# ShangtongZhang/DistributedES

Measured on NVIDIA H100. Metric: nes_policy_evals_per_sec, higher is better.
Workload: dtype f16x3 (split-fp16 operands ~ f32, f32 accumulate)

## Files before the change

### distributedes_b200/csrc/des_eval_tc.cu

```cuda
#include "des_common.cuh"
#include "des_tc.cuh"

namespace des {

using namespace tc;

constexpr int kK1 = 32;
constexpr int kMaxA = 8;
constexpr int kProdWGs = 2;
constexpr int kProdThreads = 128 * kProdWGs;
constexpr int kTcThreads = kProdThreads + 256;
constexpr int kConsWarps = 8;
template <int H, bool X3, int NA>
__host__ __device__ constexpr uint32_t prod_regs() { return (H == 256 && X3 && NA == 8) ? 40u : 56u; }
template <int H, bool X3, int NA>
__host__ __device__ constexpr uint32_t cons_regs() { return (((65536u / kTcThreads) & ~7u) * kTcThreads - kProdThreads * prod_regs<H, X3, NA>()) / 256u & ~7u; }
static_assert(cons_regs<256, true, 4>() == 200 && cons_regs<256, true, 8>() == 216, "register split");

#ifdef DES_EVAL_TRACE
enum { TR_WAIT, TR_MMA, TR_SYNC, TR_EPI, TR_GEN, TR_OTHER, TR_N };
#define DES_TRACE_INIT uint32_t tr_[TR_N] = {}; long long tr_t = clock64(), tr_0 = tr_t;
#define DES_TRACE(k) do { const long long t_ = clock64(); tr_[k] += (uint32_t)(t_ - tr_t); tr_t = t_; } while (0)
#define DES_TRACE_PRINT(role, members)                                                                                \
    if (blockIdx.x < 2 && lane == 0)                                                                                  \
        printf("DES_TRACE cta=%d warp=%d role=%s members=%d wait=%u mma=%u sync=%u epi=%u gen=%u other=%u total=%u\n", \
               (int)blockIdx.x, warp, role, members, tr_[TR_WAIT], tr_[TR_MMA], tr_[TR_SYNC], tr_[TR_EPI], tr_[TR_GEN],  \
               tr_[TR_OTHER], (uint32_t)(clock64() - tr_0))
#else
#define DES_TRACE_INIT
#define DES_TRACE(k)
#define DES_TRACE_PRINT(role, members)
#endif

template <int H, bool X3>
struct TcCfg {
    static constexpr int NCH = H / 64;
    static constexpr int KAT = H / 64;
    static constexpr int KS2 = H / 16;
    static constexpr int PLANES = X3 ? 2 : 1;
    static constexpr int CHUNK_BYTES = PLANES * KAT * 8192;
    static constexpr int W1_BYTES = PLANES * H * 128;
    static constexpr int SMALL_FLOATS = 2 * H + kMaxA * H + kMaxA;
    enum { BAR_W2_FULL = 0, BAR_W2_EMPTY = 2, BAR_W1_FULL = 4, BAR_W1_EMPTY = 5, BAR_SMALL_EMPTY = 6, NBARS = 8 };
    static constexpr size_t OFF_W1 = 2 * (size_t)CHUNK_BYTES;
    static constexpr size_t OFF_SMALL = OFF_W1 + W1_BYTES;
    static constexpr size_t OFF_FIT = OFF_SMALL + 2 * (size_t)SMALL_FLOATS * sizeof(float);
    static constexpr size_t OFF_CNT = OFF_FIT + 2 * kConsWarps * sizeof(float);
    static constexpr size_t OFF_BAR = (OFF_CNT + 2 * sizeof(uint32_t) + 7) & ~(size_t)7;
    static constexpr size_t SMEM = 1024 + OFF_BAR + NBARS * sizeof(uint64_t);
    static_assert(SMEM <= 227 * 1024, "eval_tc_kernel: shared memory over the 227 KB per-block limit");
    static_assert(SMALL_FLOATS * sizeof(float) % 16 == 0, "small-array buffers must stay float4 aligned");
};

struct TcArgs {
    float *fitness;
    const float *theta, *obs, *target;
    const des_state *state;
    Layout L;
    int T, n_pass;
    float sigma, clip, neg2ln2_sigma2;
    PhiloxKey key;
    uint32_t gen;
    uint64_t member_offset;
    int64_t n_local;
    uint8_t *cache;
};

__device__ __forceinline__ float perturbed1(const float *__restrict__ theta, int j, float sigma, uint32_t member,
                                            uint32_t gen, const PhiloxKey &key) {
    const float4 z = noise_quad((uint32_t)(j >> 2), member, gen, kStreamNesEps, key);
    const int e = j & 3;
    const float zz = e == 0 ? z.x : (e == 1 ? z.y : (e == 2 ? z.z : z.w));
    return __fmaf_rn(sigma, zz, __ldg(theta + j));
}

template <bool kMirror>
__device__ __forceinline__ float4 member_quad(uint32_t q, uint32_t member, uint32_t gen, const PhiloxKey &key,
                                              float neg2ln2_sigma2, float4 base, float sgn) {
    if (!kMirror) return perturbed_quad(q, member, gen, kStreamNesEps, key, neg2ln2_sigma2, base);
    const uint4 x = philox4x32(q, member, gen, kStreamNesEps, key);
    const BmParts a = box_muller_parts(x.x, x.y, neg2ln2_sigma2, key.one_bits);
    const BmParts b = box_muller_parts(x.z, x.w, neg2ln2_sigma2, key.one_bits);
    const float ra = a.nr * sgn, rb = b.nr * sgn;
    return make_float4(__fmaf_rn(ra, a.c, base.x), __fmaf_rn(ra, a.s, base.y), __fmaf_rn(rb, b.c, base.z),
                       __fmaf_rn(rb, b.s, base.w));
}

template <bool X3>
__device__ __forceinline__ void octet(const float (&w)[8], uint4 &hi, uint4 &lo) {
    if (X3) {
        split_h2(w[0], w[1], hi.x, lo.x); split_h2(w[2], w[3], hi.y, lo.y);
        split_h2(w[4], w[5], hi.z, lo.z); split_h2(w[6], w[7], hi.w, lo.w);
    } else {
        hi = make_uint4(pack_h2(w[0], w[1]), pack_h2(w[2], w[3]), pack_h2(w[4], w[5]), pack_h2(w[6], w[7]));
        lo = hi;
    }
}

template <bool X3>
__device__ __forceinline__ void load_x(uint32_t (&xh)[2][4], uint32_t (&xl)[2][4], const float *__restrict__ obs, int d0,
                                       int ra, int lane) {
#pragma unroll
    for (int ks = 0; ks < 2; ++ks) {
#pragma unroll
        for (int i = 0; i < 4; ++i) {
            const int row = ra + (i & 1) * 8, k = ks * 16 + (i >> 1) * 8 + (lane & 3) * 2;
            const float v0 = k < d0 ? __ldg(obs + (int64_t)row * d0 + k) : 0.f;
            const float v1 = k + 1 < d0 ? __ldg(obs + (int64_t)row * d0 + k + 1) : 0.f;
            if (X3) split_h2(v0, v1, xh[ks][i], xl[ks][i]);
            else xh[ks][i] = pack_h2(v0, v1);
        }
    }
}

template <int H, bool X3, int CL, int NA, bool kMirror>
__device__ __forceinline__ void eval_tc_body(const TcArgs &a) {
    using C = TcCfg<H, X3>;
    extern __shared__ __align__(1024) uint8_t smem_raw[];
    uint8_t *smem = reinterpret_cast<uint8_t *>((reinterpret_cast<uintptr_t>(smem_raw) + 1023) & ~(uintptr_t)1023);
    uint8_t *w2buf = smem;
    uint8_t *w1 = smem + C::OFF_W1;
    float *small_buf = reinterpret_cast<float *>(smem + C::OFF_SMALL);
    float *fit_part = reinterpret_cast<float *>(smem + C::OFF_FIT);
    uint32_t *fit_cnt = reinterpret_cast<uint32_t *>(smem + C::OFF_CNT);
    const uint32_t bars = smem_u32(smem + C::OFF_BAR);
    auto bar = [&](int k) { return bars + 8u * (uint32_t)k; };

    const int tid = threadIdx.x, warp = tid >> 5, lane = tid & 31;
    const uint32_t rank = CL == 2 ? cluster_ctarank() : 0u;
    const Layout L = a.L;
    const uint32_t gen = generation_word(a.state, a.gen);
    const int64_t first = blockIdx.x / CL, stride = gridDim.x / CL;

    constexpr uint32_t kW2Copy = (64 / CL) * 128, kW2Copies = C::PLANES * C::KAT;
    constexpr uint32_t kW1Copy = (H / CL) * 128, kW1Copies = C::PLANES;
    static_assert(CL * kW2Copies * kW2Copy == C::CHUNK_BYTES && CL * kW1Copies * kW1Copy == C::W1_BYTES,
                  "the two halves must make up the whole tile, or a full barrier never completes");
    static_assert(kW2Copy % 16 == 0 && kW1Copy % 16 == 0, "bulk copies move multiples of 16 bytes");
    static_assert(kW2Copies * kW2Copy < (1u << 20) && kW1Copies * kW1Copy < (1u << 20), "mbarrier tx-count range");

    if (tid == 0) {
        for (int s = 0; s < 2; ++s) {
            mbar_init(bar(C::BAR_W2_FULL + s), 1);
            mbar_init(bar(C::BAR_W2_EMPTY + s), kConsWarps * CL);
            mbar_init(bar(C::BAR_SMALL_EMPTY + s), kTcThreads - kProdThreads);
        }
        mbar_init(bar(C::BAR_W1_FULL), 1);
        mbar_init(bar(C::BAR_W1_EMPTY), kConsWarps * CL);
        fit_cnt[0] = fit_cnt[1] = 0u;
        fence_barrier_init();
    }
    if (CL == 2) cluster_sync_relaxed();
    __syncthreads();
    const uint32_t peer_bars = CL == 2 ? map_cluster(bars, rank ^ 1u) : 0u;
    auto release_all = [&](int k) {
        mbar_arrive(bar(k));
        if (CL == 2) mbar_arrive_remote(peer_bars + 8u * (uint32_t)k);
    };

    if (warp < 4 * kProdWGs) {
        setmaxnreg_dec<prod_regs<H, X3, NA>()>();
        DES_TRACE_INIT
        const int ptid = tid;
        uint8_t *const cache = (a.cache && a.n_pass > 1) ? a.cache + (size_t)blockIdx.x * C::NCH * C::CHUNK_BYTES : nullptr;
        auto put = [&](uint8_t *base, uint32_t off, uint32_t lo_off, const uint4 &hi, const uint4 &lo) {
            *reinterpret_cast<uint4 *>(base + off) = hi;
            if (X3) *reinterpret_cast<uint4 *>(base + lo_off + off) = lo;
        };
        auto publish = [&](int k, uint32_t base, uint32_t bytes, uint32_t ncopy, uint32_t step) {
            fence_proxy_async_cta();
            named_bar_sync(1, kProdThreads);
            if (ptid == 0) {
                if (CL == 2) {
                    mbar_expect_tx(bar(k), ncopy * bytes);
                    const uint32_t peer_bar = map_cluster(bar(k), rank ^ 1u);
                    for (uint32_t j = 0; j < ncopy; ++j) {
                        const uint32_t src = base + j * step + rank * bytes;
                        bulk_copy_to_peer(map_cluster(src, rank ^ 1u), src, bytes, peer_bar);
                    }
                } else {
                    mbar_arrive(bar(k));
                }
            }
        };
        constexpr int kOct = H / 8;
        constexpr int kRows = 64 / CL;
        auto gen_chunk = [&](uint32_t member, float sgn, int c, int pass, int buf) {
            uint8_t *dst = w2buf + buf * C::CHUNK_BYTES;
            uint8_t *mirror = cache ? cache + (size_t)c * C::CHUNK_BYTES : nullptr;
            for (int idx = ptid; idx < kRows * kOct; idx += kProdThreads) {
                const int rr = (int)rank * kRows + idx / kOct, o = idx % kOct;
                const uint32_t off = (uint32_t)((o >> 3) * 8192 + rr * 128 + (((o & 7) ^ (rr & 7)) << 4));
                uint4 hi, lo;
                if (mirror && pass > 0) {
                    hi = *reinterpret_cast<const uint4 *>(mirror + off);
                    if (X3) lo = *reinterpret_cast<const uint4 *>(mirror + C::KAT * 8192 + off);
                    else lo = hi;
                } else {
                    const int j0 = L.off_w2 + (c * 64 + rr) * H + o * 8;
                    const float4 p0 = member_quad<kMirror>((uint32_t)(j0 >> 2), member, gen, a.key, a.neg2ln2_sigma2,
                                                           __ldg(reinterpret_cast<const float4 *>(a.theta + j0)), sgn);
                    const float4 p1 = member_quad<kMirror>((uint32_t)(j0 >> 2) + 1, member, gen, a.key, a.neg2ln2_sigma2,
                                                           __ldg(reinterpret_cast<const float4 *>(a.theta + j0 + 4)), sgn);
                    const float w[8] = {p0.x, p0.y, p0.z, p0.w, p1.x, p1.y, p1.z, p1.w};
                    octet<X3>(w, hi, lo);
                    if (mirror) {
                        *reinterpret_cast<uint4 *>(mirror + off) = hi;
                        if (X3) *reinterpret_cast<uint4 *>(mirror + C::KAT * 8192 + off) = lo;
                    }
                }
                put(dst, off, C::KAT * 8192, hi, lo);
            }
        };

        uint32_t q = 0;
        int i = 0;
        for (int64_t m = first; m < a.n_local; m += stride, ++i) {
            const uint32_t member = noise_word(a.member_offset + (uint64_t)m, kMirror);
            const float sgn = member_sigma(a.member_offset + (uint64_t)m, kMirror, 1.0f);
            float *small = small_buf + (i & 1) * C::SMALL_FLOATS;
            if (i >= 2) mbar_wait(bar(C::BAR_SMALL_EMPTY + (i & 1)), ((i >> 1) - 1) & 1);
            DES_TRACE(TR_WAIT);
            for (int k = ptid; k < H / 4; k += kProdThreads) {
                const float4 v1 = member_quad<kMirror>((uint32_t)((L.off_b1 >> 2) + k), member, gen, a.key, a.neg2ln2_sigma2,
                                                       __ldg(reinterpret_cast<const float4 *>(a.theta + L.off_b1) + k), sgn);
                const float4 v2 = member_quad<kMirror>((uint32_t)((L.off_b2 >> 2) + k), member, gen, a.key, a.neg2ln2_sigma2,
                                                       __ldg(reinterpret_cast<const float4 *>(a.theta + L.off_b2) + k), sgn);
                const float bsc = X3 ? kTwoLog2e : 1.0f;
                reinterpret_cast<float4 *>(small)[k] = make_float4(v1.x * bsc, v1.y * bsc, v1.z * bsc, v1.w * bsc);
                reinterpret_cast<float4 *>(small + H)[k] = make_float4(v2.x * bsc, v2.y * bsc, v2.z * bsc, v2.w * bsc);
            }
            for (int k = ptid; k < L.A * H / 4; k += kProdThreads)
                reinterpret_cast<float4 *>(small + 2 * H)[k] =
                    member_quad<kMirror>((uint32_t)((L.off_w3 >> 2) + k), member, gen, a.key, a.neg2ln2_sigma2,
                                         __ldg(reinterpret_cast<const float4 *>(a.theta + L.off_w3) + k), sgn);
            for (int k = L.A * H + ptid; k < H * kMaxA; k += kProdThreads) small[2 * H + k] = 0.f;
            if (ptid < kMaxA)
                small[2 * H + kMaxA * H + ptid] = ptid < L.A ? perturbed1(a.theta, L.off_b3 + ptid, sgn * a.sigma, member, gen, a.key) : 0.f;
            DES_TRACE(TR_GEN);
            if (i >= 1) mbar_wait(bar(C::BAR_W1_EMPTY), (i - 1) & 1);
            DES_TRACE(TR_WAIT);
            for (int idx = ptid; idx < (H / CL) * 4; idx += kProdThreads) {
                const int n = (int)rank * (H / CL) + (idx >> 2), c8 = idx & 3;
                float w[8];
                if ((L.d0 & 3) == 0) {
#pragma unroll
                    for (int hq = 0; hq < 2; ++hq) {
                        const int k = c8 * 8 + hq * 4;
                        float4 v = make_float4(0.f, 0.f, 0.f, 0.f);
                        if (k < L.d0) {
                            const int j = L.off_w1 + n * L.d0 + k;
                            v = member_quad<kMirror>((uint32_t)(j >> 2), member, gen, a.key, a.neg2ln2_sigma2,
                                                     __ldg(reinterpret_cast<const float4 *>(a.theta + j)), sgn);
                        }
                        w[4 * hq] = v.x; w[4 * hq + 1] = v.y; w[4 * hq + 2] = v.z; w[4 * hq + 3] = v.w;
                    }
                } else {
#pragma unroll
                    for (int e = 0; e < 8; ++e) {
                        const int k = c8 * 8 + e;
                        w[e] = (k < L.d0) ? perturbed1(a.theta, L.off_w1 + n * L.d0 + k, sgn * a.sigma, member, gen, a.key) : 0.f;
                    }
                }
                uint4 hi, lo;
                octet<X3>(w, hi, lo);
                put(w1, (uint32_t)(n * 128 + ((c8 ^ (n & 7)) << 4)), H * 128, hi, lo);
            }
            DES_TRACE(TR_GEN);
            publish(C::BAR_W1_FULL, smem_u32(w1), kW1Copy, kW1Copies, H * 128);
            DES_TRACE(TR_SYNC);
            for (int pass = 0; pass < a.n_pass; ++pass) {
                for (int c = 0; c < C::NCH; ++c, ++q) {
                    const int s = (int)(q & 1u);
                    if (q >= 2) mbar_wait(bar(C::BAR_W2_EMPTY + s), ((q >> 1) - 1) & 1u);
                    DES_TRACE(TR_WAIT);
                    gen_chunk(member, sgn, c, pass, s);
                    DES_TRACE(TR_GEN);
                    publish(C::BAR_W2_FULL + s, smem_u32(w2buf + s * C::CHUNK_BYTES), kW2Copy, kW2Copies, 8192);
                    DES_TRACE(TR_SYNC);
                }
            }
        }
        if (CL == 2) {
            for (uint32_t t = q > 2u ? q - 2u : 0u; t < q; ++t) mbar_wait(bar(C::BAR_W2_EMPTY + (int)(t & 1u)), (t >> 1) & 1u);
            if (i >= 1) mbar_wait(bar(C::BAR_W1_EMPTY), (i - 1) & 1);
        }
        DES_TRACE_PRINT("producer", i);
    } else {
        setmaxnreg_inc<cons_regs<H, X3, NA>()>();
        DES_TRACE_INIT
        const int cwarp = warp - 4 * kProdWGs, cw = cwarp >> 2;
        const int r_in_tile = cw * 64 + (cwarp & 3) * 16 + (lane >> 2);
        const int cq = (lane & 3) * 2;
        uint32_t q = 0;
        int i = 0;
        for (int64_t m = first; m < a.n_local; m += stride, ++i) {
            const float *small = small_buf + (i & 1) * C::SMALL_FLOATS;
            const float *b1 = small, *b2 = small + H, *w3 = small + 2 * H, *b3 = small + 2 * H + kMaxA * H;
            mbar_wait(bar(C::BAR_W1_FULL), (uint32_t)i & 1u);
            DES_TRACE(TR_WAIT);

            float sq = 0.f;
            for (int pass = 0; pass < a.n_pass; ++pass) {
                const int tile = pass * CL + (int)rank;
                const int ra = tile * 128 + r_in_tile;
                uint32_t h1h[C::KS2][4], h1l[X3 ? C::KS2 : 1][4];
                {
                    uint32_t xh[2][4], xl[2][4];
                    load_x<X3>(xh, xl, a.obs, L.d0, ra, lane);
                    DES_TRACE(TR_OTHER);
#pragma unroll
                    for (int c = 0; c < C::NCH; ++c) {
                        float d[32];
#pragma unroll
                        for (int k = 0; k < 32; ++k) d[k] = 0.f;
                        wgmma_fence();
#pragma unroll
                        for (int ks = 0; ks < 2; ++ks) {
                            const uint32_t bh = smem_u32(w1) + c * 8192 + ks * 32;
                            wgmma_rs_n64(d, xh[ks], smem_desc_sw128(bh), ks > 0);
                            if (X3) {
                                wgmma_rs_n64(d, xl[ks], smem_desc_sw128(bh), 1);
                                wgmma_rs_n64(d, xh[ks], smem_desc_sw128(bh + H * 128), 1);
                            }
                        }
                        wgmma_commit();
                        wgmma_wait<0>();
                        fence_regs(d);
                        DES_TRACE(TR_MMA);
                        if (c == C::NCH - 1 && pass == a.n_pass - 1 && lane == 0) release_all(C::BAR_W1_EMPTY);
                        DES_TRACE(TR_SYNC);
#pragma unroll
                        for (int j = 0; j < 8; ++j) {
                            const float2 b = *reinterpret_cast<const float2 *>(b1 + c * 64 + j * 8 + cq);
                            const int s = c * 4 + (j >> 1), e = (j & 1) * 2;
#pragma unroll
                            for (int r = 0; r < 2; ++r) {
                                const float v0 = d[4 * j + 2 * r], v1 = d[4 * j + 2 * r + 1];
                                if (X3) split_h2(tanh_acc_b(v0, b.x), tanh_acc_b(v1, b.y), h1h[s][e + r], h1l[s][e + r]);
                                else h1h[s][e + r] = pack_h2(tanh_fast(v0 + b.x), tanh_fast(v1 + b.y));
                            }
                        }
                        DES_TRACE(TR_EPI);
                    }
                }
                float act[NA][2];
#pragma unroll
                for (int k = 0; k < NA; ++k) act[k][0] = act[k][1] = 0.f;
                for (int c = 0; c < C::NCH; ++c, ++q) {
                    const int st = (int)(q & 1u);
                    mbar_wait(bar(C::BAR_W2_FULL + st), (q >> 1) & 1u);
                    DES_TRACE(TR_WAIT);
                    const uint32_t bbase = smem_u32(w2buf + st * C::CHUNK_BYTES);
                    float d[32];
#pragma unroll
                    for (int k = 0; k < 32; ++k) d[k] = 0.f;
                    wgmma_fence();
#pragma unroll
                    for (int s = 0; s < C::KS2; ++s) {
                        const uint32_t bh = bbase + (s >> 2) * 8192 + (s & 3) * 32;
                        wgmma_rs_n64(d, h1h[s], smem_desc_sw128(bh), s > 0);
                        if (X3) {
                            wgmma_rs_n64(d, h1l[s], smem_desc_sw128(bh), 1);
                            wgmma_rs_n64(d, h1h[s], smem_desc_sw128(bh + C::KAT * 8192), 1);
                        }
                    }
                    wgmma_commit();
                    wgmma_wait<0>();
                    fence_regs(d);
                    DES_TRACE(TR_MMA);
                    if (lane == 0) release_all(C::BAR_W2_EMPTY + st);
                    DES_TRACE(TR_SYNC);
#pragma unroll
                    for (int j = 0; j < 8; ++j) {
                        const int n = c * 64 + j * 8 + cq;
                        const float2 b = *reinterpret_cast<const float2 *>(b2 + n);
#pragma unroll
                        for (int r = 0; r < 2; ++r) {
                            float h0, h1;
                            if (X3) {
                                h0 = tanh_acc_b(d[4 * j + 2 * r], b.x);
                                h1 = tanh_acc_b(d[4 * j + 2 * r + 1], b.y);
                            } else {
                                h0 = tanh_fast(d[4 * j + 2 * r] + b.x);
                                h1 = tanh_fast(d[4 * j + 2 * r + 1] + b.y);
                            }
#pragma unroll
                            for (int k = 0; k < NA; ++k) {
                                if (k < L.A) {
                                    const float2 w = *reinterpret_cast<const float2 *>(w3 + k * H + n);
                                    act[k][r] = __fmaf_rn(h1, w.y, __fmaf_rn(h0, w.x, act[k][r]));
                                }
                            }
                        }
                    }
                    DES_TRACE(TR_EPI);
                }
#pragma unroll
                for (int k = 0; k < NA; ++k) {
#pragma unroll
                    for (int r = 0; r < 2; ++r) {
                        act[k][r] += __shfl_xor_sync(0xffffffffu, act[k][r], 1);
                        act[k][r] += __shfl_xor_sync(0xffffffffu, act[k][r], 2);
                    }
                }
                if ((lane & 3) == 0) {
#pragma unroll
                    for (int r = 0; r < 2; ++r) {
                        const int t = ra + 8 * r;
#pragma unroll
                        for (int k = 0; k < NA; ++k) {
                            if (k < L.A) {
                                float v = act[k][r] + b3[k];
                                v = clip_keep_nan(v, a.clip);
                                const float dd = v - __ldg(a.target + (int64_t)t * L.A + k);
                                sq = __fmaf_rn(dd, dd, sq);
                            }
                        }
                    }
                }
            }
#pragma unroll
            for (int o = 16; o > 0; o >>= 1) sq += __shfl_xor_sync(0xffffffffu, sq, o);
            if (lane == 0) {
                float *part = fit_part + (i & 1) * kConsWarps;
                part[cwarp] = sq;
                __threadfence_block();
                if (atomicAdd(fit_cnt + (i & 1), 1u) == kConsWarps - 1) {
                    __threadfence_block();
                    double f = 0.0;
                    for (int w = 0; w < kConsWarps; ++w) f += (double)reinterpret_cast<volatile float *>(part)[w];
                    fit_cnt[i & 1] = 0u;
                    if (CL == 2) atomicAdd(a.fitness + m, (float)(-f));
                    else a.fitness[m] = (float)(-f);
                }
            }
            mbar_arrive(bar(C::BAR_SMALL_EMPTY + (i & 1)));
            DES_TRACE(TR_OTHER);
        }
        DES_TRACE_PRINT("consumer", i);
    }
}

template <int H, bool X3, int CL, int NA>
__global__ void __launch_bounds__(kTcThreads, 1) eval_tc_kernel(TcArgs a) { eval_tc_body<H, X3, CL, NA, false>(a); }

template <int H, bool X3, int CL, int NA>
__global__ void __launch_bounds__(kTcThreads, 1) eval_tc_mirrored_kernel(TcArgs a) { eval_tc_body<H, X3, CL, NA, true>(a); }

template <int H, bool X3, int CL, int NA, bool kMirror>
static int launch_tc(TcArgs &a, cudaStream_t st) {
    using C = TcCfg<H, X3>;
    const auto kernel = kMirror ? eval_tc_mirrored_kernel<H, X3, CL, NA> : eval_tc_kernel<H, X3, CL, NA>;
    a.n_pass = a.T / 128 / CL;
    int dev = 0, sms = 132;
    DES_CUDA(cudaGetDevice(&dev));
    DES_CUDA(cudaDeviceGetAttribute(&sms, cudaDevAttrMultiProcessorCount, dev));
    if (CL == 2) {
        DES_CUDA(cudaFuncSetAttribute(kernel, cudaFuncAttributeMaxDynamicSharedMemorySize, (int)C::SMEM));
        DES_CUDA(cudaMemsetAsync(a.fitness, 0, (size_t)a.n_local * sizeof(float), st));
        const int64_t clusters = a.n_local < sms / 2 ? a.n_local : sms / 2;
        cudaLaunchConfig_t cfg = {};
        cfg.gridDim = dim3((unsigned)(2 * clusters));
        cfg.blockDim = dim3(kTcThreads);
        cfg.dynamicSmemBytes = C::SMEM;
        cfg.stream = st;
        cudaLaunchAttribute attr[1];
        attr[0].id = cudaLaunchAttributeClusterDimension;
        attr[0].val.clusterDim.x = 2;
        attr[0].val.clusterDim.y = 1;
        attr[0].val.clusterDim.z = 1;
        cfg.attrs = attr;
        cfg.numAttrs = 1;
        DES_CUDA(cudaLaunchKernelEx(&cfg, kernel, a));
        DES_LAUNCH_CHECK("eval_tc_kernel");
        return DES_OK;
    }
    const int64_t grid = a.n_local < sms ? a.n_local : sms;
    return launch_smem("eval_tc_kernel", kernel, (unsigned)grid, kTcThreads, C::SMEM, st, a);
}

template <int H, bool X3, bool kMirror>
static int launch_tc_m(TcArgs &a, cudaStream_t st) {
    const bool even = (a.T / 128) % 2 == 0;
    if (a.L.A <= 4) return even ? launch_tc<H, X3, 2, 4, kMirror>(a, st) : launch_tc<H, X3, 1, 4, kMirror>(a, st);
    return even ? launch_tc<H, X3, 2, kMaxA, kMirror>(a, st) : launch_tc<H, X3, 1, kMaxA, kMirror>(a, st);
}

template <int H, bool X3>
static int launch_tc_h(TcArgs &a, bool mirrored, cudaStream_t st) {
    return mirrored ? launch_tc_m<H, X3, true>(a, st) : launch_tc_m<H, X3, false>(a, st);
}

static int tc_passes(int T) { const int tiles = T / 128; return tiles % 2 == 0 ? tiles / 2 : tiles; }

size_t eval_tc_workspace_bytes(des_dims dims, int precision) {
    const int H = dims.hidden;
    if (!(H == 64 || H == 128 || H == 256) || dims.tape_len % 128 != 0 || tc_passes(dims.tape_len) <= 1) return 0;
    int dev = 0, sms = 132;
    if (cudaGetDevice(&dev) != cudaSuccess || cudaDeviceGetAttribute(&sms, cudaDevAttrMultiProcessorCount, dev) != cudaSuccess) {
        cudaGetLastError();
        sms = 132;
    }
    return (size_t)sms * (size_t)H * H * 2 * (precision == DES_FWD_F16X3 ? 2 : 1);
}

int eval_tc_launch(float *fitness, const float *theta, const float *obs, const float *target, des_dims dims,
                   double sigma, double clip, uint64_t seed, uint64_t generation, const des_state *state,
                   int64_t member_offset, int64_t n_local, int precision, void *workspace, size_t workspace_bytes,
                   bool mirrored, cudaStream_t st) {
    const int H = dims.hidden;
    if (!(H == 64 || H == 128 || H == 256) || dims.state_dim > kK1 || dims.action_dim > kMaxA || dims.tape_len % 128 != 0) {
        set_error("des_nes_eval(tensor): needs hidden in {64,128,256}, state_dim <= %d, action_dim <= %d, tape_len %% 128 == 0 "
                  "(got d0=%d H=%d A=%d T=%d); use DES_FWD_FP32 for other shapes", kK1, kMaxA, dims.state_dim, H,
                  dims.action_dim, dims.tape_len);
        return DES_ERR_UNSUPPORTED;
    }
    if (((uintptr_t)theta & 15) != 0) {
        set_error("des_nes_eval(tensor): theta_dev must be 16-byte aligned");
        return DES_ERR_INVALID_ARGUMENT;
    }
    TcArgs a;
    a.fitness = fitness; a.theta = theta; a.obs = obs; a.target = target; a.state = state;
    a.L = Layout(dims.state_dim, H, dims.action_dim);
    a.T = dims.tape_len;
    a.sigma = (float)sigma; a.clip = (float)clip;
    a.neg2ln2_sigma2 = kNeg2Ln2 * (float)sigma * (float)sigma;
    a.key = make_philox_key(seed); a.gen = (uint32_t)generation;
    a.member_offset = (uint64_t)member_offset; a.n_local = n_local;
    const bool x3 = precision == DES_FWD_F16X3;
    const size_t need = eval_tc_workspace_bytes(dims, precision);
    a.cache = (need > 0 && workspace && workspace_bytes >= need && ((uintptr_t)workspace & 15) == 0) ? (uint8_t *)workspace : nullptr;
    switch (H) {
        case 64: return x3 ? launch_tc_h<64, true>(a, mirrored, st) : launch_tc_h<64, false>(a, mirrored, st);
        case 128: return x3 ? launch_tc_h<128, true>(a, mirrored, st) : launch_tc_h<128, false>(a, mirrored, st);
        default: return x3 ? launch_tc_h<256, true>(a, mirrored, st) : launch_tc_h<256, false>(a, mirrored, st);
    }
}

}
```

### distributedes_b200/csrc/des_tc.cuh

```cuda
#pragma once
#include <cuda_fp16.h>
#include <stdint.h>

namespace des {
namespace tc {

__device__ __forceinline__ uint32_t smem_u32(const void *p) { return (uint32_t)__cvta_generic_to_shared(p); }

__device__ __forceinline__ void mbar_init(uint32_t bar, uint32_t count) {
    asm volatile("mbarrier.init.shared::cta.b64 [%0], %1;" ::"r"(bar), "r"(count) : "memory");
}
__device__ __forceinline__ void fence_barrier_init() { asm volatile("fence.mbarrier_init.release.cluster;" ::: "memory"); }
__device__ __forceinline__ bool mbar_try_wait(uint32_t bar, uint32_t parity) {
    uint32_t ok;
    asm volatile(
        "{\n\t.reg .pred p;\n\t"
        "mbarrier.try_wait.parity.shared::cta.b64 p, [%1], %2, %3;\n\t"
        "selp.u32 %0, 1, 0, p;\n\t}"
        : "=r"(ok) : "r"(bar), "r"(parity), "r"(1000000u) : "memory");
    return ok != 0;
}
__device__ __forceinline__ void mbar_wait(uint32_t bar, uint32_t parity) {
    while (!mbar_try_wait(bar, parity)) {
    }
}
__device__ __forceinline__ void mbar_arrive(uint32_t bar) {
    asm volatile("mbarrier.arrive.shared::cta.b64 _, [%0];" ::"r"(bar) : "memory");
}
__device__ __forceinline__ void mbar_arrive_remote(uint32_t cbar) {
    asm volatile("mbarrier.arrive.shared::cluster.b64 _, [%0];" ::"r"(cbar) : "memory");
}
__device__ __forceinline__ void mbar_expect_tx(uint32_t bar, uint32_t bytes) {
    asm volatile("mbarrier.arrive.expect_tx.shared::cta.b64 _, [%0], %1;" ::"r"(bar), "r"(bytes) : "memory");
}
__device__ __forceinline__ void fence_proxy_async_cta() { asm volatile("fence.proxy.async.shared::cta;" ::: "memory"); }
__device__ __forceinline__ void named_bar_sync(uint32_t id, uint32_t n) {
    asm volatile("bar.sync %0, %1;" ::"r"(id), "r"(n) : "memory");
}

__device__ __forceinline__ void tma_load_2d(uint32_t dst, const void *map, int c0, int c1, uint32_t bar) {
    asm volatile(
        "cp.async.bulk.tensor.2d.shared::cluster.global.tile.mbarrier::complete_tx::bytes [%0], [%1, {%2, %3}], [%4];"
        ::"r"(dst), "l"(map), "r"(c0), "r"(c1), "r"(bar) : "memory");
}

__device__ __forceinline__ bool elect_one() {
    uint32_t pred;
    asm volatile("{\n\t.reg .pred p;\n\telect.sync _|p, 0xffffffff;\n\tselp.u32 %0, 1, 0, p;\n\t}" : "=r"(pred));
    return pred != 0;
}

__device__ __forceinline__ uint32_t cluster_ctarank() {
    uint32_t r;
    asm volatile("mov.u32 %0, %%cluster_ctarank;" : "=r"(r));
    return r;
}
__device__ __forceinline__ void cluster_sync_relaxed() {
    asm volatile("barrier.cluster.arrive.relaxed.aligned;\n\tbarrier.cluster.wait.aligned;" ::: "memory");
}
__device__ __forceinline__ uint32_t map_cluster(uint32_t saddr, uint32_t rank) {
    uint32_t ra;
    asm volatile("mapa.shared::cluster.u32 %0, %1, %2;" : "=r"(ra) : "r"(saddr), "r"(rank));
    return ra;
}
__device__ __forceinline__ void bulk_copy_to_peer(uint32_t cdst, uint32_t src, uint32_t bytes, uint32_t cbar) {
    asm volatile("cp.async.bulk.shared::cluster.shared::cta.mbarrier::complete_tx::bytes [%0], [%1], %2, [%3];"
                 ::"r"(cdst), "r"(src), "r"(bytes), "r"(cbar) : "memory");
}

template <uint32_t N>
__device__ __forceinline__ void setmaxnreg_inc() { asm volatile("setmaxnreg.inc.sync.aligned.u32 %0;" ::"n"(N)); }
template <uint32_t N>
__device__ __forceinline__ void setmaxnreg_dec() { asm volatile("setmaxnreg.dec.sync.aligned.u32 %0;" ::"n"(N)); }

__device__ __forceinline__ uint64_t smem_desc_sw128(uint32_t saddr) {
    return (uint64_t)((saddr & 0x3FFFFu) >> 4) | (1ull << 16) | (64ull << 32) | (1ull << 62);
}
__device__ __forceinline__ void wgmma_fence() { asm volatile("wgmma.fence.sync.aligned;" ::: "memory"); }
__device__ __forceinline__ void wgmma_commit() { asm volatile("wgmma.commit_group.sync.aligned;" ::: "memory"); }
template <int N>
__device__ __forceinline__ void wgmma_wait() { asm volatile("wgmma.wait_group.sync.aligned %0;" ::"n"(N) : "memory"); }
template <int N>
__device__ __forceinline__ void fence_regs(float (&d)[N]) {
#pragma unroll
    for (int i = 0; i < N; ++i) asm volatile("" : "+f"(d[i])::"memory");
}

#define DES_F8(d, o) "+f"(d[o + 0]), "+f"(d[o + 1]), "+f"(d[o + 2]), "+f"(d[o + 3]), "+f"(d[o + 4]), "+f"(d[o + 5]), \
                     "+f"(d[o + 6]), "+f"(d[o + 7])

__device__ __forceinline__ void wgmma_rs_n64(float (&d)[32], const uint32_t (&a)[4], uint64_t b_desc, uint32_t acc) {
    asm volatile(
        "{\n\t.reg .pred p;\n\tsetp.ne.b32 p, %37, 0;\n\t"
        "wgmma.mma_async.sync.aligned.m64n64k16.f32.f16.f16 "
        "{%0, %1, %2, %3, %4, %5, %6, %7, %8, %9, %10, %11, %12, %13, %14, %15, "
        "%16, %17, %18, %19, %20, %21, %22, %23, %24, %25, %26, %27, %28, %29, %30, %31}, "
        "{%32, %33, %34, %35}, %36, p, 1, 1, 0;\n\t}"
        : DES_F8(d, 0), DES_F8(d, 8), DES_F8(d, 16), DES_F8(d, 24)
        : "r"(a[0]), "r"(a[1]), "r"(a[2]), "r"(a[3]), "l"(b_desc), "r"(acc));
}
__device__ __forceinline__ void wgmma_ss_n128(float (&d)[64], uint64_t a_desc, uint64_t b_desc, uint32_t acc) {
    asm volatile(
        "{\n\t.reg .pred p;\n\tsetp.ne.b32 p, %66, 0;\n\t"
        "wgmma.mma_async.sync.aligned.m64n128k16.f32.f16.f16 "
        "{%0, %1, %2, %3, %4, %5, %6, %7, %8, %9, %10, %11, %12, %13, %14, %15, "
        "%16, %17, %18, %19, %20, %21, %22, %23, %24, %25, %26, %27, %28, %29, %30, %31, "
        "%32, %33, %34, %35, %36, %37, %38, %39, %40, %41, %42, %43, %44, %45, %46, %47, "
        "%48, %49, %50, %51, %52, %53, %54, %55, %56, %57, %58, %59, %60, %61, %62, %63}, "
        "%64, %65, p, 1, 1, 0, 0;\n\t}"
        : DES_F8(d, 0), DES_F8(d, 8), DES_F8(d, 16), DES_F8(d, 24), DES_F8(d, 32), DES_F8(d, 40), DES_F8(d, 48),
          DES_F8(d, 56)
        : "l"(a_desc), "l"(b_desc), "r"(acc));
}
#undef DES_F8

__device__ __forceinline__ uint32_t pack_h2(float lo, float hi) {
    const __half2 h = __floats2half2_rn(lo, hi);
    return *reinterpret_cast<const uint32_t *>(&h);
}
__device__ __forceinline__ void split_h2(float a, float b, uint32_t &hi, uint32_t &lo) {
    const __half2 h = __floats2half2_rn(a, b);
    const float2 hf = __half22float2(h);
    const __half2 l = __floats2half2_rn(a - hf.x, b - hf.y);
    hi = *reinterpret_cast<const uint32_t *>(&h);
    lo = *reinterpret_cast<const uint32_t *>(&l);
}

constexpr float kTwoLog2e = 2.8853900817779268f;
__device__ __forceinline__ float tanh_acc_b(float v, float bs) {
    float e, r;
    asm("ex2.approx.ftz.f32 %0, %1;" : "=f"(e) : "f"(__fmaf_rn(v, kTwoLog2e, bs)));
    asm("rcp.approx.ftz.f32 %0, %1;" : "=f"(r) : "f"(1.0f + e));
    return __fmaf_rn(-2.0f, r, 1.0f);
}

__device__ __forceinline__ float tanh_fast(float x) {
    float y;
    asm("tanh.approx.f32 %0, %1;" : "=f"(y) : "f"(x));
    return y;
}

}
}
```

Baseline: 2.977 million.

## Alternate wgmma issue between consumer warpgroups with named-barrier turn passing

Adds a ping-pong schedule between the two consumer warpgroups for H=256 split-fp16 configs. Each warpgroup waits on a named barrier before issuing its wgmma batch and signals the other once the batch is committed, so tensor-core issue alternates while the other warpgroup runs its tanh/split epilogue. The aim is to overlap epilogue math with MMA and reduce contention. The cost is extra barrier waits, and any mismatch in turn counts between the warpgroups could serialize them or deadlock.

```diff
diff --git a/distributedes_b200/csrc/des_eval_tc.cu b/distributedes_b200/csrc/des_eval_tc.cu
--- a/distributedes_b200/csrc/des_eval_tc.cu
+++ b/distributedes_b200/csrc/des_eval_tc.cu
@@ -18,14 +18,14 @@
 static_assert(cons_regs<256, true, 4>() == 200 && cons_regs<256, true, 8>() == 216, "register split");
 
 #ifdef DES_EVAL_TRACE
-enum { TR_WAIT, TR_MMA, TR_SYNC, TR_EPI, TR_GEN, TR_OTHER, TR_N };
+enum { TR_WAIT, TR_TURN, TR_MMA, TR_SYNC, TR_EPI, TR_GEN, TR_OTHER, TR_N };
 #define DES_TRACE_INIT uint32_t tr_[TR_N] = {}; long long tr_t = clock64(), tr_0 = tr_t;
 #define DES_TRACE(k) do { const long long t_ = clock64(); tr_[k] += (uint32_t)(t_ - tr_t); tr_t = t_; } while (0)
-#define DES_TRACE_PRINT(role, members)                                                                                \
-    if (blockIdx.x < 2 && lane == 0)                                                                                  \
-        printf("DES_TRACE cta=%d warp=%d role=%s members=%d wait=%u mma=%u sync=%u epi=%u gen=%u other=%u total=%u\n", \
-               (int)blockIdx.x, warp, role, members, tr_[TR_WAIT], tr_[TR_MMA], tr_[TR_SYNC], tr_[TR_EPI], tr_[TR_GEN],  \
-               tr_[TR_OTHER], (uint32_t)(clock64() - tr_0))
+#define DES_TRACE_PRINT(role, members)                                                                                 \
+    if (blockIdx.x < 2 && lane == 0)                                                                                   \
+        printf("DES_TRACE cta=%d warp=%d role=%s members=%d wait=%u turn=%u mma=%u sync=%u epi=%u gen=%u other=%u "    \
+               "total=%u\n", (int)blockIdx.x, warp, role, members, tr_[TR_WAIT], tr_[TR_TURN], tr_[TR_MMA], tr_[TR_SYNC], \
+               tr_[TR_EPI], tr_[TR_GEN], tr_[TR_OTHER], (uint32_t)(clock64() - tr_0))
 #else
 #define DES_TRACE_INIT
 #define DES_TRACE(k)
@@ -113,7 +113,7 @@
     }
 }
 
-template <int H, bool X3, int CL, int NA, bool kMirror>
+template <int H, bool X3, int CL, int NA, bool kMirror, bool kTurns>
 __device__ __forceinline__ void eval_tc_body(const TcArgs &a) {
     using C = TcCfg<H, X3>;
     extern __shared__ __align__(1024) uint8_t smem_raw[];
@@ -292,6 +292,14 @@
         const int cwarp = warp - 4 * kProdWGs, cw = cwarp >> 2;
         const int r_in_tile = cw * 64 + (cwarp & 3) * 16 + (lane >> 2);
         const int cq = (lane & 3) * 2;
+        auto take_turn = [&] {
+            if (kTurns) {
+                named_bar_sync_sel<2, 3, 256>(cw);
+                DES_TRACE(TR_TURN);
+            }
+        };
+        auto pass_turn = [&] { if (kTurns) named_bar_arrive_sel<3, 2, 256>(cw); };
+        if (cw == 1) pass_turn();
         uint32_t q = 0;
         int i = 0;
         for (int64_t m = first; m < a.n_local; m += stride, ++i) {
@@ -311,6 +319,7 @@
                     DES_TRACE(TR_OTHER);
 #pragma unroll
                     for (int c = 0; c < C::NCH; ++c) {
+                        take_turn();
                         float d[32];
 #pragma unroll
                         for (int k = 0; k < 32; ++k) d[k] = 0.f;
@@ -325,6 +334,7 @@
                             }
                         }
                         wgmma_commit();
+                        pass_turn();
                         wgmma_wait<0>();
                         fence_regs(d);
                         DES_TRACE(TR_MMA);
@@ -351,6 +361,7 @@
                     const int st = (int)(q & 1u);
                     mbar_wait(bar(C::BAR_W2_FULL + st), (q >> 1) & 1u);
                     DES_TRACE(TR_WAIT);
+                    take_turn();
                     const uint32_t bbase = smem_u32(w2buf + st * C::CHUNK_BYTES);
                     float d[32];
 #pragma unroll
@@ -366,6 +377,7 @@
                         }
                     }
                     wgmma_commit();
+                    pass_turn();
                     wgmma_wait<0>();
                     fence_regs(d);
                     DES_TRACE(TR_MMA);
@@ -438,15 +450,23 @@
             mbar_arrive(bar(C::BAR_SMALL_EMPTY + (i & 1)));
             DES_TRACE(TR_OTHER);
         }
+        if (cw == 0) take_turn();
         DES_TRACE_PRINT("consumer", i);
     }
 }
 
+template <int H, bool X3>
+__host__ __device__ constexpr bool turns() { return X3 && H == 256; }
+
 template <int H, bool X3, int CL, int NA>
-__global__ void __launch_bounds__(kTcThreads, 1) eval_tc_kernel(TcArgs a) { eval_tc_body<H, X3, CL, NA, false>(a); }
+__global__ void __launch_bounds__(kTcThreads, 1) eval_tc_kernel(TcArgs a) {
+    eval_tc_body<H, X3, CL, NA, false, turns<H, X3>()>(a);
+}
 
 template <int H, bool X3, int CL, int NA>
-__global__ void __launch_bounds__(kTcThreads, 1) eval_tc_mirrored_kernel(TcArgs a) { eval_tc_body<H, X3, CL, NA, true>(a); }
+__global__ void __launch_bounds__(kTcThreads, 1) eval_tc_mirrored_kernel(TcArgs a) {
+    eval_tc_body<H, X3, CL, NA, true, turns<H, X3>()>(a);
+}
 
 template <int H, bool X3, int CL, int NA, bool kMirror>
 static int launch_tc(TcArgs &a, cudaStream_t st) {
diff --git a/distributedes_b200/csrc/des_tc.cuh b/distributedes_b200/csrc/des_tc.cuh
--- a/distributedes_b200/csrc/des_tc.cuh
+++ b/distributedes_b200/csrc/des_tc.cuh
@@ -36,6 +36,16 @@
 __device__ __forceinline__ void fence_proxy_async_cta() { asm volatile("fence.proxy.async.shared::cta;" ::: "memory"); }
 __device__ __forceinline__ void named_bar_sync(uint32_t id, uint32_t n) {
     asm volatile("bar.sync %0, %1;" ::"r"(id), "r"(n) : "memory");
+}
+template <uint32_t ID0, uint32_t ID1, uint32_t N>
+__device__ __forceinline__ void named_bar_sync_sel(uint32_t sel) {
+    asm volatile("{\n\t.reg .pred p;\n\tsetp.eq.u32 p, %0, 0;\n\t@p bar.sync %1, %3;\n\t@!p bar.sync %2, %3;\n\t}"
+                 ::"r"(sel), "n"(ID0), "n"(ID1), "n"(N) : "memory");
+}
+template <uint32_t ID0, uint32_t ID1, uint32_t N>
+__device__ __forceinline__ void named_bar_arrive_sel(uint32_t sel) {
+    asm volatile("{\n\t.reg .pred p;\n\tsetp.eq.u32 p, %0, 0;\n\t@p bar.arrive %1, %3;\n\t@!p bar.arrive %2, %3;\n\t}"
+                 ::"r"(sel), "n"(ID0), "n"(ID1), "n"(N) : "memory");
 }
 
 __device__ __forceinline__ void tma_load_2d(uint32_t dst, const void *map, int c0, int c1, uint32_t bar) {
```

After: 3.007 million, median of 6. 1.01x the previous value.
